# HyeonwooNoh/VQA-Transfer-ExternalData

Hardware: AMD Instinct MI355X
Metric: VQA train samples/sec (img+question) at bs512 (higher is better)
Workload: dtype f32

## Files before the change

include/vqa_hot.h:

```cpp
#ifndef VQA_HOT_H
#define VQA_HOT_H

#include <stdint.h>

#ifdef __cplusplus
extern "C" {
#endif

#define VQA_HOT_ABI_VERSION 5

enum {
    VQA_OK = 0,
    VQA_ERR_ARG = -1,
    VQA_ERR_ALIGN = -2,
    VQA_ERR_LAUNCH = -3,
    VQA_ERR_UNSUPPORTED = -4,
    VQA_ERR_WORKSPACE = -5
};

int vqa_hot_version(void);
const char* vqa_hot_error_string(int code);

int vqa_gather_features(const float* table, const int32_t* nbox_table, const int64_t* idx,
                        float* V, int32_t* nb, int B, int R, int D, int64_t N, void* stream);
// ... 8 lines not shown
int vqa_gru_unpack_dwx_bias(const float* dwx, float* gwg, float* gwc, float* gbg, float* gbc, int W, int H, void* stream);
int vqa_set_deterministic(int on);
int vqa_embed_bwd(const float* dx_tm, const int32_t* q, float* dE, int B, int T, int W, int Vq, void* stream);
int vqa_embed_bwd_len(const float* dx_tm, const int32_t* q, const int32_t* len, float* dE, int B, int T, int W,
                      int Vq, void* stream);
int vqa_embed_bwd_len_det(const float* dx_tm, const int32_t* q, const int32_t* len, float* dE, int B, int T, int W,
                          int Vq, int deterministic, void* stream);

int vqa_gemm_f32(int transA, int transB, int M, int N, int K, const float* A, int lda, const float* B,
                 int ldb, float* C, int ldc, const float* bias, const float* D, int ldd, int split_k,
                 float* workspace, int64_t workspace_floats, void* stream);
int vqa_gemm_f32_ex(int transA, int transB, int M, int N, int K, const float* A, int lda, const float* B,
                    int ldb, float* C, int ldc, const float* bias, const float* D, int ldd, int split_k,
                    float* workspace, int64_t workspace_floats, int max_blocks, void* stream);
int vqa_gemm_f32_gather(int M, int N, int K, const float* table, int lda, const int64_t* idx, int R,
                        int64_t n_samples_in_table, const float* B, int ldb, float* C, int ldc, const float* bias,
                        float* gathered_out, int ldg, void* stream);
int vqa_gemm_set_max_blocks(int n);
int vqa_gemm_set_order(int order);
int64_t vqa_gemm_workspace_floats(int transA, int transB, int M, int N, int K, int split_k);
int vqa_gemm_set_config(int cfg);
int vqa_gemm_set_gru_config(int cfg);
int vqa_gemm_set_tall_config(int cfg);

int vqa_ln_set_fast(int on);
int vqa_ln_relu_fwd(const float* pre, const float* gamma, const float* beta, const uint8_t* keepmask,
                    float keep_prob, float* y, float* mean, float* rstd, int G, int rows, int N, void* stream);
int vqa_ln_relu_bwd(const float* dy, const float* pre, const float* mean, const float* rstd,
                    const float* gamma, const float* beta, const uint8_t* keepmask, float keep_prob,
                    float* dpre, float* part_dgamma, float* part_dbeta, float* part_dbias, int G, int rows,
                    int N, void* stream);
int vqa_ln_act_fwd(const float* pre, const float* gamma, const float* beta, const uint8_t* keepmask, float keep_prob,
                   float* y, float* mean, float* rstd, int G, int rows, int N, int act, void* stream);
int vqa_ln_act_bwd(const float* dy, const float* pre, const float* mean, const float* rstd, const float* gamma,
                   const float* beta, const uint8_t* keepmask, float keep_prob, float* dpre, float* part_dgamma,
                   float* part_dbeta, float* part_dbias, int G, int rows, int N, int act, void* stream);
int vqa_ln_pair_mul_supported(int N, const void* const* ptrs, int n_ptrs);
int vqa_ln_pair_mul_fwd(const float* pre_a, const float* pre_b, const float* gamma_a, const float* beta_a, const float* gamma_b,
                        const float* beta_b, float* y_a, float* y_b, float* z, float* mean_a, float* rstd_a, float* mean_b,
                        float* rstd_b, int G, int N, void* stream);
int vqa_ln_pair_mul_bwd(const float* dz, const float* add_b, const float* pre_a, const float* pre_b, const float* mean_a,
                        const float* rstd_a, const float* mean_b, const float* rstd_b, const float* gamma_a, const float* beta_a,
                        const float* gamma_b, const float* beta_b, float* dpre_a, float* dpre_b, float* part_dgamma_a,
                        float* part_dbeta_a, float* part_dbias_a, float* part_dgamma_b, float* part_dbeta_b, float* part_dbias_b,
                        int G, int N, void* stream);
int vqa_tanh_fwd(const float* x, float* y, int64_t n, void* stream);
// ... 593 lines not shown
```

vqa-transfer-externaldata_amd/_lib.py:

```python
from __future__ import annotations

import ctypes as C
import os

_HERE = os.path.dirname(os.path.abspath(__file__))
_LIB_PATH = os.path.join(_HERE, "libvqahot.so")


class VqaHotError(RuntimeError):
    pass


def lib_path():
    return _LIB_PATH


class Dims(C.Structure):
    _fields_ = [("B", C.c_int32), ("R", C.c_int32), ("D", C.c_int32), ("H", C.c_int32), ("T", C.c_int32),
                ("W", C.c_int32), ("A", C.c_int32), ("Vq", C.c_int32), ("N_img", C.c_int64),
                ("model_type", C.c_int32), ("keep_att", C.c_float), ("keep_joint", C.c_float),
                ("inv_global_batch", C.c_float), ("flags", C.c_int32),
                ("num_marginal", C.c_int32), ("ent_cols", C.c_int32), ("extra_weight", C.c_float),
                ("map_dim", C.c_int32), ("La", C.c_int32)]

# ... 131 lines not shown


_P, _I, _L, _F, _U = C.c_void_p, C.c_int, C.c_int64, C.c_float, C.c_uint64

SIGNATURES = {
    "vqa_hot_version": (_I, []),
    "vqa_hot_error_string": (C.c_char_p, [_I]),
    "vqa_gather_features": (_I, [_P, _P, _P, _P, _P, _I, _I, _I, _L, _P]),
    "vqa_gather_features_bf16": (_I, [_P, _P, _P, _P, _P, _I, _I, _I, _L, _P]),
    "vqa_embed_fwd": (_I, [_P, _P, _P, _I, _I, _I, _I, _P]),
    "vqa_gru_pack_wx": (_I, [_P, _P, _P, _P, _P, _P, _I, _I, _P]),
    "vqa_gru_unpack_dwx": (_I, [_P, _P, _P, _I, _I, _P]),
    "vqa_embed_fwd_ld": (_I, [_P, _P, _P, _I, _I, _I, _I, _I, _P]),
    "vqa_gru_unpack_dwx_bias": (_I, [_P, _P, _P, _P, _P, _I, _I, _P]),
    "vqa_embed_bwd": (_I, [_P, _P, _P, _I, _I, _I, _I, _P]),
    "vqa_embed_bwd_len": (_I, [_P, _P, _P, _P, _I, _I, _I, _I, _P]),
    "vqa_embed_bwd_len_det": (_I, [_P, _P, _P, _P, _I, _I, _I, _I, _I, _P]),
    "vqa_set_deterministic": (_I, [_I]),
    "vqa_gemm_f32": (_I, [_I, _I, _I, _I, _I, _P, _I, _P, _I, _P, _I, _P, _P, _I, _I, _P, _L, _P]),
    "vqa_gemm_workspace_floats": (_L, [_I, _I, _I, _I, _I, _I]),
    "vqa_gemm_f32_ex": (_I, [_I, _I, _I, _I, _I, _P, _I, _P, _I, _P, _I, _P, _P, _I, _I, _P, _L, _I, _P]),
    "vqa_gemm_f32_gather": (_I, [_I, _I, _I, _P, _I, _P, _I, _L, _P, _I, _P, _I, _P, _P, _I, _P]),
    "vqa_gemm_set_tall_config": (_I, [_I]),
    "vqa_gemm_set_max_blocks": (_I, [_I]),
    "vqa_gemm_set_order": (_I, [_I]),
    "vqa_gemm_set_config": (_I, [_I]),
    "vqa_conv_set_config": (_I, [_I]),
    "vqa_gemm_set_gru_config": (_I, [_I]),
    "vqa_gru_seq_fwd": (_I, [_P, _P, _P, _P, _P, _P, _P, _P, _P, _I, _I, _I, _P]),
    "vqa_gru_seq_fwd_persistent": (_I, [_P, _P, _P, _P, _P, _P, _P, _P, _P, _I, _I, _I, _P, _P]),
    "vqa_gru_fwd_persistent_supported": (_I, [_I, _I, _I]),
    "vqa_gru_persistent_sync_bytes": (_L, []),
    "vqa_gru_set_persistent": (_I, [_I]),
    "vqa_gru_persistent_set_census": (_I, [_P]),
    "vqa_gru_seq_fwd_ws": (_I, [_P, _P, _P, _P, _P, _P, _P, _P, _P, _I, _I, _I, _P, _P]),
    "vqa_gru_seq_fwd_ws_ex": (_I, [_P, _P, _P, _P, _P, _P, _P, _P, _P, _I, _I, _I, _I, _P, _P]),
    "vqa_gru_ws_supported": (_I, [_I, _I, _I]),
    "vqa_gru_seq_bwd_ws": (_I, [_P, _P, _P, _P, _P, _P, _P, _P, _P, _P, _I, _I, _I, _P, _P]),
    "vqa_gru_seq_bwd_ws_ex": (_I, [_P, _P, _P, _P, _P, _P, _P, _P, _P, _P, _I, _I, _I, _I, _P, _P]),
    "vqa_gru_ws_bwd_supported": (_I, [_I, _I, _I]),
    "vqa_gru_ws_workspace_bytes": (_L, [_I]),
    "vqa_gru_ws_set_mode": (_I, [_I]),
    "vqa_gru_ws_set_form": (_I, [_I]),
    "vqa_gru_ws_set_stamps": (_I, [_P]),
    "vqa_gru_seq_fwd_rows": (_I, [_P, _P, _P, _P, _P, _P, _P, _P, _P, _I, _I, _I, _I, _I, _P]),
    "vqa_gru_seq_bwd_rows": (_I, [_P, _P, _P, _P, _P, _P, _P, _P, _P, _P, _I, _I, _I, _I, _I, _P]),
# ... 204 lines not shown
```

vqa-transfer-externaldata_amd/csrc/fusion_model.hip:

```cpp
#include <stdlib.h>
#include <string.h>

#include <string>
#include <vector>

#include "gru_encoder.h"
#include "keep_launch.h"

namespace {

inline bool has_tuned_head(int mt) { return mt == VQA_MODEL_VQA_ALL2 || mt == VQA_MODEL_VQA_ALL; }
inline bool train_loss_masked(int mt) { return mt != VQA_MODEL_STANDARD; }
inline bool bf16_routed(int mt) { return mt == VQA_MODEL_VLMAP_ANSWER || mt == VQA_MODEL_STANDARD; }
inline bool feat16(const vqa_dims_t& d) { return (d.flags & VQA_FLAG_BF16_FEATURES) != 0; }

void legacy_vqa_layout(Layout& L, const vqa_dims_t& d, int64_t& gw);

Layout make_layout(const vqa_dims_t& d) {
    Layout L;
    const int64_t B = d.B, R = d.R, D = d.D, H = d.H, T = d.T, W = d.W, A = d.A;
    L.add("V_ft", B * R * D, feat16(d) ? 2 : 4);
    L.add("num_V_ft", B);
    L.add("pre_v", B * R * H);
    L.add("v_linear_v", B * R * H);
    L.add("mean_v", B); L.add("rstd_v", B);
    const int64_t Wp = x_stride(W);
    L.add("x_tm", T * B * Wp);
    L.add("xp", T * B * 3 * H);
// ... 156 lines not shown
int g_h0skip_mode = -1;
inline int h0skip_mode() {
    if (g_h0skip_mode < 0) {
        const char* e = getenv("VQA_HOT_GRU_H0SKIP");
        g_h0skip_mode = e == nullptr ? 1 : (atoi(e) & 3);
    }
    return g_h0skip_mode;
}
int side_max_blocks() {
    static int v = -1;
    if (v < 0) {
        const char* e = getenv("VQA_HOT_SIDE_BLOCKS");
        v = e ? atoi(e) : 0;
    }
    return v;
}
int gather_mode(const vqa_dims_t* dims) {
    static int env = -2;
    if (env == -2) {
        const char* e = getenv("VQA_HOT_GATHER");
        env = e == nullptr ? -1 : (strcmp(e, "fused") == 0 ? 1 : 0);
    }
    if (env >= 0) return env;
    return (dims->flags & VQA_FLAG_FUSED_GATHER) ? 1 : 0;
}

struct Side {
    hipStream_t s = nullptr;
    hipEvent_t fork = nullptr, join = nullptr;
    bool ok = false, tried = false;
};
Side& side_stream() {
    static Side sd[64];
    int dev = 0;
    (void)hipGetDevice(&dev);
    Side& x = sd[dev & 63];
    if (!x.tried) {
        x.tried = true;
        const char* env = getenv("VQA_HOT_OVERLAP");
        if (env != nullptr && env[0] == '1') {
            x.ok = hipStreamCreateWithFlags(&x.s, hipStreamNonBlocking) == hipSuccess &&
                   hipEventCreateWithFlags(&x.fork, hipEventDisableTiming) == hipSuccess &&
                   hipEventCreateWithFlags(&x.join, hipEventDisableTiming) == hipSuccess;
        }
    }
    return x;
}
// ... 372 lines not shown

    Ctx side_ctx() const { return Ctx{{L, c.ws}, d, forked ? sd->s : c.st, forked ? 1 : 0}; }
    float* const dh = c.f("d_h0");
};

int side_record(const Step& s) { return !s.forked || join_side_record(*s.sd) ? VQA_OK : VQA_ERR_LAUNCH; }
int side_wait(const Step& s) {
    return !s.forked || hipStreamWaitEvent(s.c.st, s.sd->join, 0) == hipSuccess ? VQA_OK : VQA_ERR_LAUNCH;
}

enum GruForm { GRU_WS, GRU_LIVE, GRU_CHAINS };
enum GruDir { GRU_FWD, GRU_BWD };
GruForm gru_form(GruDir dir, int64_t T, int64_t B, int64_t H, const int32_t* live_rows) {
    const bool ws_ok = gru_ws_on() && (live_rows == nullptr || (T > 0 && live_rows[T - 1] > 0));
    if (ws_ok && (dir == GRU_FWD ? vqa_gru_ws_supported((int)T, (int)B, (int)H) : vqa_gru_ws_bwd_supported((int)T, (int)B, (int)H)) == 1)
        return GRU_WS;
    return live_rows != nullptr ? GRU_LIVE : GRU_CHAINS;
}


void fwd_visual_plan(Step& s) {
    s.sd = &side_stream();
    s.forked = fork_side(s.c, *s.sd);
    s.fuse_gather = !(s.d.flags & VQA_FLAG_BF16_GEMM) && gather_mode(&s.d) == 1 && (s.D % 32 == 0) && (s.H % 4 == 0) &&
                    vqa_aligned16(s.bt->table);
    s.visual_late = !s.forked && visual_late_enabled();
}

int fwd_visual(const Step& s) {
    const Ctx cv = s.side_ctx();
    const vqa_params_t* P = s.P;
    const vqa_batch_t* bt = s.bt;
    const int64_t B = s.B, R = s.R, D = s.D, H = s.H;
    {
        ProbeScope ps("gather", cv.st);
        if (feat16(s.d))
            TRY(vqa_gather_features_bf16(reinterpret_cast<const uint16_t*>(bt->table), bt->nbox_table, bt->image_idx,
                                         cv.u16("V_ft"), cv.i32("num_V_ft"), (int)B, (int)R, (int)D, s.d.N_img, cv.st));
        else
            TRY(vqa_gather_features(bt->table, bt->nbox_table, bt->image_idx, s.fuse_gather ? nullptr : cv.f("V_ft"),
                                    cv.i32("num_V_ft"), (int)B, (int)R, (int)D, s.d.N_img, cv.st));
    }
    if (s.fuse_gather) {
        {
            ProbeScope ps("v_linear_v.fwd_gemm", cv.st);
            TRY(vqa_gemm_f32_gather((int)(B * R), (int)H, (int)D, bt->table, (int)D, bt->image_idx, (int)R, s.d.N_img,
                                    P->v_linear_v.w, (int)H, cv.f("pre_v"), (int)H, P->v_linear_v.b, cv.f("V_ft"), (int)D,
// ... 609 lines not shown
```

vqa-transfer-externaldata_amd/csrc/gemm_args.h:

```cpp
#pragma once
#include <hip/hip_runtime.h>
#include <stdint.h>

struct GemmArgs {
    int M, N, K;
    const float* A; int lda;
    const float* B; int ldb;
    float* C; int ldc;
    const float* bias;
    const float* D; int ldd;
    int k_per_split;
    int64_t slab_stride;
    int vecA, vecB;
    int tiles_m, tiles_n, nsplit;
    int m_fastest;
    unsigned a_bytes, b_bytes;
    const float* scale;
    int relu;
    int Hi, Wi, Ci, Ho, Wo, cstride, pad_t, pad_l, kw;
    int conv_taps;
    int vec_epi;
    const int64_t* g_idx; int g_R; int64_t g_N; float* g_out; int g_ldo;
};

enum { EPI_PLAIN = 0, EPI_GATES = 1, EPI_CAND = 2, EPI_BWD_RH = 3, EPI_BWD_DH = 4 };
struct EpiArgs {
    int H, t, ldo;
    const int32_t* len;
    const float* h_prev;
    const float* i0;
    const float* i1;
    float* o0;
    float* o1;
    float* o2;
};

GemmArgs vqa_gemm_make_args(int M, int N, int K, const float* A, int lda, const float* B, int ldb, float* C, int ldc,
                            const float* bias, const float* D, int ldd);
int vqa_gru_step_launch(int epi, int cfg, const GemmArgs& a, const EpiArgs& ep, hipStream_t st);
int vqa_gru_rs_launch(int epi, const GemmArgs& a, const EpiArgs& ep, hipStream_t st);
```

vqa-transfer-externaldata_amd/csrc/gemm_f32.hip:

```cpp

#include "vqa_common.h"
#include "gemm_args.h"
#include <cstdio>
#include <cstdlib>

#ifndef VQA_GEMM_STAGGER
#define VQA_GEMM_STAGGER 1
#endif

typedef float f32x16 __attribute__((ext_vector_type(16)));
typedef unsigned int u32x4 __attribute__((ext_vector_type(4)));

#if defined(VQA_DBG_STAMPS)
__device__ unsigned long long* g_dbg_stamps = nullptr;
#define DBG_STAMP(i) do { if (threadIdx.x == 0) dbg_t[i] = __builtin_amdgcn_s_memrealtime(); } while (0)
#else
#define DBG_STAMP(i) do {} while (0)
#endif

namespace {


__device__ __forceinline__ int xcd_remap(int lin, int total) {
    const int q = total >> 3, r = total & 7;
// ... 153 lines not shown
                    const int k = idx / QPR, rq = (idx % QPR) * 4;
                    *reinterpret_cast<float4*>(s + k * BR + rq) = reg[i];
                }
            }
        }
    }
};

template <int BR, int BK, bool KC>
constexpr int tile_floats() { return KC ? BR * (BK + 4) : BK * BR; }

template <int BR, int BK, bool KC>
__device__ __forceinline__ float4 frag4(const float* s, int r0, int c, int lane) {
    const int i = lane & 31, h = lane >> 5;
    if (KC) {
        return *reinterpret_cast<const float4*>(s + (r0 + i) * (BK + 4) + c * 8 + h * 4);
    } else {
        const float* p = s + (c * 8 + h * 4) * BR + r0 + i;
        return make_float4(p[0], p[BR], p[2 * BR], p[3 * BR]);
    }
}

template <int BM, int BN, int WM, int WN, int WGK, int BK, int DEEP, bool A_KC, bool B_KC, int EPI, bool CONV = false,
          bool EDGE = false, int NT = 256, bool GATHER = false>
__global__ __launch_bounds__(NT, (CONV && NT == 256) ? 4 : 1) void gemm_f32_kernel(GemmArgs p, EpiArgs ep) {
    static_assert(!GATHER || (A_KC && DEEP == 0 && !CONV && !EDGE && EPI == EPI_PLAIN), "row-gathered A: plain NN/NT tiles");
    constexpr int TM = WM / 32, TN = WN / 32;
    constexpr int WAVES_M = BM / WM, WAVES_N = BN / WN;
    static_assert(WAVES_M * WAVES_N * WGK * 64 == NT, "one 32x32-tiled wave per (m, n, k-group) slot");
    static_assert((BK / 8) % WGK == 0, "k chunks split evenly over the k wave groups");
    constexpr int A_FL = tile_floats<BM, BK, A_KC>();
    constexpr int B_FL = tile_floats<BN, BK, B_KC>();
    extern __shared__ __attribute__((aligned(16))) float smem[];

    if (EPI != EPI_PLAIN) __builtin_amdgcn_s_setprio(3);
#if defined(VQA_DBG_STAMPS)
    unsigned long long dbg_t[8] = {0, 0, 0, 0, 0, 0, 0, 0};
    if (threadIdx.x == 0) dbg_t[5] = __builtin_amdgcn_s_memtime();
#endif
    DBG_STAMP(0);
    const int lane = threadIdx.x & 63, wave = threadIdx.x >> 6;
    const int wk = wave / (WAVES_M * WAVES_N);
    const int wm = (wave / WAVES_N) % WAVES_M, wn = wave % WAVES_N;
    const int tiles_mn = p.tiles_m * p.tiles_n;
    const int total = tiles_mn * p.nsplit;
    for (int lin = blockIdx.x; lin < total; lin += gridDim.x) {
    const int tile = xcd_remap(lin, total);
    const int bz = tile / tiles_mn, bmn = tile - bz * tiles_mn;
    const int m0 = (p.m_fastest ? bmn % p.tiles_m : bmn / p.tiles_n) * BM;
// ... 93 lines not shown
        Stager<BN, BK, B_KC, NT> sb;
        constexpr int NVA = Stager<BM, BK, A_KC, NT>::NV;
        int iy0[NVA], ix0[NVA], pix[NVA];
        if (CONV) {
#pragma unroll
            for (int i = 0; i < NVA; ++i) {
                const int idx = threadIdx.x + i * NT;
                const int m = m0 + idx / (BK / 4);
                pix[i] = -1; iy0[i] = ix0[i] = 0;
                if (idx < BM * (BK / 4) && m < p.M) {
                    const int hw = p.Ho * p.Wo;
                    const int b = m / hw, r = m - b * hw;
                    const int oy = r / p.Wo, ox = r - oy * p.Wo;
                    iy0[i] = oy * p.cstride - p.pad_t;
                    ix0[i] = ox * p.cstride - p.pad_l;
                    pix[i] = b * p.Hi * p.Wi;
                }
            }
        }
        const float* gsrc[NVA];
        unsigned gdst[NVA];
        const bool g_store = GATHER && p.g_out != nullptr && n0 == 0;
        const __amdgpu_buffer_rsrc_t rsG = __builtin_amdgcn_make_buffer_rsrc(
            p.g_out, 0, GATHER && p.g_out != nullptr ? (int)(((int64_t)(p.M - 1) * p.g_ldo + p.K) * 4) : 0, 0x00020000);
        if (GATHER) {
#pragma unroll
            for (int i = 0; i < NVA; ++i) {
                const int idx = threadIdx.x + i * NT;
                const int row = idx / (BK / 4), kq = (idx % (BK / 4)) * 4;
                const int m = m0 + row, mc = min(m, p.M - 1);
                const int smp = mc / p.g_R, reg_row = mc - smp * p.g_R;
                int64_t src = p.g_idx[smp];
                src = src < 0 ? 0 : (src >= p.g_N ? p.g_N - 1 : src);
                gsrc[i] = p.A + (src * p.g_R + reg_row) * (int64_t)p.lda + kq;
                gdst[i] = (m < p.M) ? (unsigned)(((int64_t)m * p.g_ldo + kq) * 4) : Stager<BM, BK, A_KC, NT>::OOB;
            }
        }
        auto load_a = [&](int k0) {
            if (GATHER) sa.load_ptr(gsrc, k0 - kbeg);
            else if (CONV) sa.load_conv(rsA, iy0, ix0, pix, k0, p.Hi, p.Wi, p.Ci, p.kw);
            else if (EDGE) sa.load(p.A, p.lda, m0, k0, p.M, kend, va);
            else sa.load_fast(rsA, p.lda, m0, k0, p.M, kend);
        };
        auto load_b = [&](int k0) {
            if (EDGE) sb.load(p.B, p.ldb, n0, k0, p.N, kend, vb);
            else sb.load_fast(rsB, p.ldb, n0, k0, p.N, kend);
        };
        if (nt > 0) {
            load_a(kbeg);
            load_b(kbeg);
            sa.store(L0);
            sb.store(L0 + A_FL);
            if (g_store) sa.store_buf(rsG, gdst, 0u);
        }
        __syncthreads();
        int t = 0;
        if (CONV && p.conv_taps <= 32 && p.Ci % BK == 0) {
            unsigned cbase[NVA], cmask[NVA];
            const int kh = p.conv_taps / p.kw;
#pragma unroll
            for (int i = 0; i < NVA; ++i) {
                const int idx = threadIdx.x + i * NT;
// ... 18 lines not shown
            };
            if (c0 >= p.Ci) { c0 = 0; tap = 1; if (++kx == p.kw) { kx = 0; ++ky; } }
            for (; t + 2 < nt; t += 2) {
                sa.load_conv_full(rsA, cbase, cmask, (unsigned)(((ky * p.Wi + kx) * p.Ci + c0) * 4), 1u << tap);
                sb.load_full(rsB, ob);
                ob += stepB; advance();
                __builtin_amdgcn_sched_barrier(0);
                compute_tile(L0, L0 + A_FL);
                __builtin_amdgcn_sched_barrier(0);
                sa.store(L1);
                sb.store(L1 + A_FL);
                __syncthreads();
                sa.load_conv_full(rsA, cbase, cmask, (unsigned)(((ky * p.Wi + kx) * p.Ci + c0) * 4), 1u << tap);
                sb.load_full(rsB, ob);
                ob += stepB; advance();
                __builtin_amdgcn_sched_barrier(0);
                compute_tile(L1, L1 + A_FL);
                __builtin_amdgcn_sched_barrier(0);
                sa.store(L0);
                sb.store(L0 + A_FL);
                __syncthreads();
            }
        }
        if (!CONV && !EDGE) {
            sa.init_full(p.lda, m0, kbeg, p.M);
            sb.init_full(p.ldb, n0, kbeg, p.N);
            const unsigned stepA = (unsigned)(A_KC ? BK : BK * p.lda) * 4u;
            const unsigned stepB = (unsigned)(B_KC ? BK : BK * p.ldb) * 4u;
            const int nfull = (kend - kbeg) / BK;
            unsigned oa = stepA, ob = stepB;
            constexpr bool STAG = (NT == 512) && !GATHER && EPI == EPI_PLAIN && (VQA_GEMM_STAGGER != 0) &&
                                  ((WM == 32 && WN == 32 && BK == 32 && BM + BN == 192) || (BM == 128 && BN == 128 && BK == 16));
            const bool stag_wg = STAG && nfull >= 16;
            if (stag_wg && wave >= 4) {
                sa.load_full(rsA, oa); sb.load_full(rsB, ob);
                oa += stepA; ob += stepB;
                for (; t + 3 < nfull; t += 2) {
                    sa.store(L1); sb.store(L1 + A_FL);
                    sa.load_full(rsA, oa); sb.load_full(rsB, ob);
                    oa += stepA; ob += stepB;
                    __builtin_amdgcn_sched_barrier(0);
                    compute_tile(L0, L0 + A_FL);
                    __builtin_amdgcn_sched_barrier(0);
                    __syncthreads();
                    sa.store(L0); sb.store(L0 + A_FL);
                    sa.load_full(rsA, oa); sb.load_full(rsB, ob);
                    oa += stepA; ob += stepB;
                    __builtin_amdgcn_sched_barrier(0);
                    compute_tile(L1, L1 + A_FL);
                    __builtin_amdgcn_sched_barrier(0);
                    __syncthreads();
                }
                sa.store(L1); sb.store(L1 + A_FL);
                __builtin_amdgcn_sched_barrier(0);
                compute_tile(L0, L0 + A_FL);
                __builtin_amdgcn_sched_barrier(0);
                __syncthreads();
                ++t;
            } else if (stag_wg) {
                for (; t + 3 < nfull; t += 2) {
                    sa.load_full(rsA, oa); sb.load_full(rsB, ob);
                    oa += stepA; ob += stepB;
                    __builtin_amdgcn_sched_barrier(0);
                    compute_tile(L0, L0 + A_FL);
                    __builtin_amdgcn_sched_barrier(0);
                    sa.store(L1); sb.store(L1 + A_FL);
                    __syncthreads();
                    sa.load_full(rsA, oa); sb.load_full(rsB, ob);
                    oa += stepA; ob += stepB;
                    __builtin_amdgcn_sched_barrier(0);
                    compute_tile(L1, L1 + A_FL);
                    __builtin_amdgcn_sched_barrier(0);
                    sa.store(L0); sb.store(L0 + A_FL);
                    __syncthreads();
                }
                sa.load_full(rsA, oa); sb.load_full(rsB, ob);
                __builtin_amdgcn_sched_barrier(0);
                compute_tile(L0, L0 + A_FL);
                __builtin_amdgcn_sched_barrier(0);
                sa.store(L1); sb.store(L1 + A_FL);
                __syncthreads();
                ++t;
            }
            for (; !stag_wg && t + 2 < nfull; t += 2) {
                if (GATHER) sa.load_ptr(gsrc, (t + 1) * BK); else sa.load_full(rsA, oa);
                sb.load_full(rsB, ob);
                oa += stepA; ob += stepB;
                __builtin_amdgcn_sched_barrier(0);
                compute_tile(L0, L0 + A_FL);
                __builtin_amdgcn_sched_barrier(0);
                sa.store(L1);
                sb.store(L1 + A_FL);
                if (g_store) sa.store_buf(rsG, gdst, (unsigned)((t + 1) * BK) * 4u);
                __syncthreads();
                if (GATHER) sa.load_ptr(gsrc, (t + 2) * BK); else sa.load_full(rsA, oa);
                sb.load_full(rsB, ob);
                oa += stepA; ob += stepB;
                __builtin_amdgcn_sched_barrier(0);
                compute_tile(L1, L1 + A_FL);
                __builtin_amdgcn_sched_barrier(0);
                sa.store(L0);
                sb.store(L0 + A_FL);
                if (g_store) sa.store_buf(rsG, gdst, (unsigned)((t + 2) * BK) * 4u);
                __syncthreads();
            }
        }
        for (; t + 1 < nt; ++t) {
            float* cur = (t & 1) ? L1 : L0;
            float* nxt = (t & 1) ? L0 : L1;
            load_a(kbeg + (t + 1) * BK);
            load_b(kbeg + (t + 1) * BK);
            __builtin_amdgcn_sched_barrier(0);
            compute_tile(cur, cur + A_FL);
            __builtin_amdgcn_sched_barrier(0);
            sa.store(nxt);
            sb.store(nxt + A_FL);
            if (g_store) sa.store_buf(rsG, gdst, (unsigned)((t + 1) * BK) * 4u);
            __syncthreads();
        }
        if (nt > 0) {
            float* cur = ((nt - 1) & 1) ? L1 : L0;
            compute_tile(cur, cur + A_FL);
            __syncthreads();
        }
    } else {
        Stager<BM, BK, A_KC, NT> sa0, sa1;
        Stager<BN, BK, B_KC, NT> sb0, sb1;
        auto ld0 = [&](int tile) {
            sa0.load_fast(rsA, p.lda, m0, kbeg + tile * BK, p.M, kend);
            sb0.load_fast(rsB, p.ldb, n0, kbeg + tile * BK, p.N, kend);
        };
        auto ld1 = [&](int tile) {
            sa1.load_fast(rsA, p.lda, m0, kbeg + tile * BK, p.M, kend);
            sb1.load_fast(rsB, p.ldb, n0, kbeg + tile * BK, p.N, kend);
        };
        auto st0 = [&]() { sa0.store(L0); sb0.store(L0 + A_FL); };
        auto st1 = [&]() { sa1.store(L1); sb1.store(L1 + A_FL); };
        if (nt > 0) ld0(0);
        if (nt > 1) ld1(1);
        if (nt > 0) st0();
        __syncthreads();
        DBG_STAMP(1);
        int t = 0;
        {
            sa0.init_full(p.lda, m0, kbeg, p.M); sa1.init_full(p.lda, m0, kbeg, p.M);
            sb0.init_full(p.ldb, n0, kbeg, p.N); sb1.init_full(p.ldb, n0, kbeg, p.N);
// ... 273 lines not shown
        unsigned long long* o = g_dbg_stamps + ((size_t)EPI * 4096 + blockIdx.x) * 8;
        for (int i = 0; i < 7; ++i) o[i] = dbg_t[i];
    }
#endif
}

__global__ __launch_bounds__(256) void splitk_reduce_kernel(const float* __restrict__ slabs, float* __restrict__ C,
                                                            int M, int N, int ldc, int S) {
    const int64_t n4 = (int64_t)M * N / 4;
    for (int64_t i = blockIdx.x * 256 + threadIdx.x; i < n4; i += (int64_t)gridDim.x * 256) {
        float4 a = reinterpret_cast<const float4*>(slabs)[i];
        for (int z = 1; z < S; ++z) {
            const float4 b = reinterpret_cast<const float4*>(slabs + (int64_t)z * M * N)[i];
            a.x += b.x; a.y += b.y; a.z += b.z; a.w += b.w;
        }
        const int64_t e = i * 4;
        const int row = (int)(e / N), col = (int)(e % N);
        float* c = C + (int64_t)row * ldc + col;
        c[0] = a.x; c[1] = a.y; c[2] = a.z; c[3] = a.w;
    }
}

template <int BM, int BN, int WM, int WN, int WGK, int BK, int DEEP, bool A_KC, bool B_KC, int EPI, bool CONV = false,
          bool EDGE = false, int NT = 256, bool GATHER = false>
int launch_one(GemmArgs a, const EpiArgs& ep, int split, hipStream_t st, int max_blocks = 0) {
    constexpr size_t tiles = 2 * (tile_floats<BM, BK, A_KC>() + tile_floats<BN, BK, B_KC>()) * sizeof(float);
    constexpr size_t red = (EPI == EPI_PLAIN) ? (size_t)(WGK - 1) * (BM / WM) * (BN / WN) * (WM / 32) * (WN / 32) * 16 * 64 * sizeof(float) : 0;
    constexpr size_t stage = (size_t)(EPI == EPI_PLAIN ? 1 : WGK) * (BM / WM) * (BN / WN) * 32 * 36 * sizeof(float);
    constexpr size_t lds = tiles > red + stage ? tiles : red + stage;
    auto kern = gemm_f32_kernel<BM, BN, WM, WN, WGK, BK, DEEP, A_KC, B_KC, EPI, CONV, EDGE, NT, GATHER>;
    static bool attr_done = false;
    if (lds > 64 * 1024 && !attr_done) {
        if (hipFuncSetAttribute(reinterpret_cast<const void*>(kern), hipFuncAttributeMaxDynamicSharedMemorySize,
                                (int)lds) != hipSuccess)
            return VQA_ERR_LAUNCH;
        attr_done = true;
    }
    a.tiles_m = (a.M + BM - 1) / BM;
    a.tiles_n = (a.N + BN - 1) / BN;
    a.nsplit = split;
    {
        const double per_xcd = (double)a.tiles_m * a.tiles_n / 8.0;
        auto foot = [&](double t_fast, double t_slow, double b_fast, double b_slow) {
            const double slow_panels = std::min(t_slow, per_xcd / t_fast + 1.0);
            const double fast_panels = std::min(t_fast, per_xcd);
            return slow_panels * b_slow + fast_panels * b_fast;
        };
// ... 94 lines not shown
        case 4: return launch_one<64, 64, 32, 32, 1, 64, false, true, BKC, EPI>(a, ep, 1, st);
        case 7: return launch_one<64, 32, 32, 32, 2, 64, false, true, BKC, EPI>(a, ep, 1, st);
        case 8: return launch_one<32, 32, 32, 32, 4, 64, false, true, BKC, EPI>(a, ep, 1, st);
        case 9: return launch_one<32, 64, 32, 32, 2, 64, false, true, BKC, EPI>(a, ep, 1, st);
        case 10: return launch_one<64, 64, 32, 32, 1, 64, true, true, BKC, EPI>(a, ep, 1, st);
        case 11: return launch_one<64, 32, 32, 32, 2, 64, true, true, BKC, EPI>(a, ep, 1, st);
        case 12: return launch_one<64, 64, 32, 32, 1, 32, true, true, BKC, EPI>(a, ep, 1, st);
        case 13: return launch_one<64, 32, 32, 32, 2, 32, true, true, BKC, EPI>(a, ep, 1, st);
        case 16: return launch_one<32, 32, 32, 32, 4, 32, true, true, BKC, EPI>(a, ep, 1, st);
        case 20: return launch_one<128, 64, 32, 32, 1, 32, 0, true, BKC, EPI, false, false, 512>(a, ep, 1, st);
        case 21: return launch_one<64, 128, 32, 32, 1, 32, 0, true, BKC, EPI, false, false, 512>(a, ep, 1, st);
        case 17: return launch_one<64, 32, 32, 32, 4, 32, 1, true, BKC, EPI, false, false, 512>(a, ep, 1, st);
        case 18:
            if (EPI == EPI_GATES) return launch_one<64, 64, 32, 32, 4, 64, 1, true, BKC, EPI, false, false, 1024>(a, ep, 1, st);
            return launch_one<64, 32, 32, 32, 8, 64, 1, true, BKC, EPI, false, false, 1024>(a, ep, 1, st);
        default: return VQA_ERR_ARG;
    }
}

inline int64_t cdiv(int64_t a, int64_t b) { return (a + b - 1) / b; }

int g_force_cfg = -1;
int g_tall_cfg = 20;
int g_max_blocks = 0;
int g_conv_cfg = -1;
int g_conv_cfg_plain = -1;

inline int tall_small_cfg() {
    static const int v = vqa_env_int("VQA_HOT_TALL_SMALL_CFG", 12);
    return v < NUM_CFG ? v : 12;
}

inline int tune_pair(const char* env, int cfg, int split) {
    const char* e = getenv(env);
    if (e != nullptr) {
        int c = 0, s = 0;
        if (sscanf(e, "%d:%d", &c, &s) == 2 && c >= 0 && c < NUM_CFG && s >= 0 && s <= 16) { cfg = c; split = s; }
    }
    return (cfg << 8) | split;
}

void choose(int tA, int tB, int M, int N, int K, int& cfg, int& split) {
    int64_t target;
    if (tA) {
        static const int tn_short = vqa_env_int("VQA_HOT_TN_SHORT_CFG", 20);
        static const int tn_mid = vqa_env_int("VQA_HOT_TN_MID_CFG", 20);
// ... 160 lines not shown
        const int grid = (int)std::min<int64_t>(cdiv(n4, 256), 2048);
        hipLaunchKernelGGL(splitk_reduce_kernel, dim3(grid), dim3(256), 0, st, workspace, C, M, N, ldc, split);
        VQA_CHECK_LAUNCH();
        return VQA_OK;
    }
    a.k_per_split = (int)cdiv(std::max(K, 1), 64) * 64;
    return launch_by_id(cfg, transA, transB, a, 1, st, max_blocks);
}

extern "C" int vqa_gemm_f32_gather(int M, int N, int K, const float* table, int lda, const int64_t* idx, int R,
                                   int64_t n_samples_in_table, const float* B, int ldb, float* C, int ldc,
                                   const float* bias, float* gathered_out, int ldg, void* stream) {
    VQA_REQUIRE(M >= 0 && N >= 0 && K > 0 && R > 0 && n_samples_in_table > 0, VQA_ERR_ARG);
    if (M == 0 || N == 0) return VQA_OK;
    VQA_REQUIRE(table && idx && B && C, VQA_ERR_ARG);
    VQA_REQUIRE(lda >= K && ldb >= N && ldc >= N && (gathered_out == nullptr || ldg >= K), VQA_ERR_ARG);
    VQA_REQUIRE(K % 32 == 0 && N % 4 == 0, VQA_ERR_UNSUPPORTED);
    VQA_REQUIRE(lda % 4 == 0 && vqa_aligned16(table) && ldb % 4 == 0 && vqa_aligned16(B) &&
                    (gathered_out == nullptr || (ldg % 4 == 0 && vqa_aligned16(gathered_out))),
                VQA_ERR_ALIGN);
    GemmArgs a = vqa_gemm_make_args(M, N, K, table, lda, B, ldb, C, ldc, bias, nullptr, 0);
    const int64_t bb = ((int64_t)(K - 1) * ldb + N) * 4;
    VQA_REQUIRE(bb < 0xFFFFFF00ll, VQA_ERR_UNSUPPORTED);
    a.a_bytes = 0;
    a.b_bytes = (unsigned)bb;
    VQA_REQUIRE(gathered_out == nullptr || ((int64_t)(M - 1) * ldg + K) * 4 < 0xFFFFFF00ll, VQA_ERR_UNSUPPORTED);
    a.g_idx = idx; a.g_R = R; a.g_N = n_samples_in_table; a.g_out = gathered_out; a.g_ldo = ldg;
    a.k_per_split = (int)cdiv(K, 64) * 64;
    const EpiArgs ep{};
    hipStream_t st = static_cast<hipStream_t>(stream);
    if (g_tall_cfg == 21)
        return launch_one<64, 128, 32, 32, 1, 32, 0, true, false, EPI_PLAIN, false, false, 512, true>(a, ep, 1, st, 0);
    return launch_one<128, 64, 32, 32, 1, 32, 0, true, false, EPI_PLAIN, false, false, 512, true>(a, ep, 1, st, 0);
}

extern "C" int vqa_gemm_set_tall_config(int cfg) {
    VQA_REQUIRE(cfg == 20 || cfg == 21, VQA_ERR_ARG);
    g_tall_cfg = cfg;
    return VQA_OK;
}

extern "C" int vqa_conv2d_nhwc(const float* x, int B, int Hi, int Wi, int Ci, const float* w, int kh, int kw, int Co,
                               int stride, int pad_t, int pad_l, int Ho, int Wo, const float* scale,
                               const float* shift, const float* residual, int relu, float* y, void* stream) {
    VQA_REQUIRE(x && w && y && B > 0 && Hi > 0 && Wi > 0 && Ci > 0 && Co > 0 && kh > 0 && kw > 0 && stride > 0 &&
                    Ho > 0 && Wo > 0,
                VQA_ERR_ARG);
    VQA_REQUIRE((int64_t)B * Ho * Wo < (1ll << 31) && (int64_t)B * Hi * Wi < (1ll << 31), VQA_ERR_ARG);
    hipStream_t st = static_cast<hipStream_t>(stream);
    const int M = B * Ho * Wo, K = kh * kw * Ci;
    const bool plain = (kh == 1 && kw == 1 && stride == 1 && pad_t == 0 && pad_l == 0 && Ho == Hi && Wo == Wi);
    GemmArgs a = vqa_gemm_make_args(M, Co, K, x, Ci, w, Co, y, Co, shift, residual, Co);
    a.scale = scale;
    a.relu = relu;
    if (plain && (shortk_mode() & 2) && Ci >= 128 && Ci <= 256 && Co >= 2 * Ci && g_conv_cfg_plain < 0 && g_force_cfg < 0 &&
        vqa_gemm_shortk_supported(M, Co, K, Ci, Co, Co) && vqa_aligned16(x) && vqa_aligned16(w) &&
// ... 35 lines not shown
```

Baseline: 164,000.

## Fuse row gather into GEMM via buffer offsets and enable by default

Adds a gather GEMM variant that loads gathered A rows through buffer-resource offsets, so the table rows share the same staggered, pipelined k-loop as the plain GEMM instead of going through per-thread pointer loads. The k-loop is moved into an include file so it can be specialised for the offset gather, pointer gather and plain paths. The default gather mode now fuses the gather into the GEMM whenever the plain heuristic would pick the same tall config, which removes the separate gather kernel and the extra pass over memory for the features. The risk is that gathered rows are scattered, so A loads coalesce less well, and the table must fit within the 32-bit buffer offset range.

```diff
diff --git a/include/vqa_hot.h b/include/vqa_hot.h
--- a/include/vqa_hot.h
+++ b/include/vqa_hot.h
@@ -54,6 +54,7 @@
 int vqa_gemm_set_config(int cfg);
 int vqa_gemm_set_gru_config(int cfg);
 int vqa_gemm_set_tall_config(int cfg);
+int vqa_gemm_set_gather_ptr(int on);
 
 int vqa_ln_set_fast(int on);
 int vqa_ln_relu_fwd(const float* pre, const float* gamma, const float* beta, const uint8_t* keepmask,
diff --git a/vqa-transfer-externaldata_amd/_lib.py b/vqa-transfer-externaldata_amd/_lib.py
--- a/vqa-transfer-externaldata_amd/_lib.py
+++ b/vqa-transfer-externaldata_amd/_lib.py
@@ -177,6 +177,7 @@
     "vqa_gemm_f32_ex": (_I, [_I, _I, _I, _I, _I, _P, _I, _P, _I, _P, _I, _P, _P, _I, _I, _P, _L, _I, _P]),
     "vqa_gemm_f32_gather": (_I, [_I, _I, _I, _P, _I, _P, _I, _L, _P, _I, _P, _I, _P, _P, _I, _P]),
     "vqa_gemm_set_tall_config": (_I, [_I]),
+    "vqa_gemm_set_gather_ptr": (_I, [_I]),
     "vqa_gemm_set_max_blocks": (_I, [_I]),
     "vqa_gemm_set_order": (_I, [_I]),
     "vqa_gemm_set_config": (_I, [_I]),
diff --git a/vqa-transfer-externaldata_amd/csrc/fusion_model.hip b/vqa-transfer-externaldata_amd/csrc/fusion_model.hip
--- a/vqa-transfer-externaldata_amd/csrc/fusion_model.hip
+++ b/vqa-transfer-externaldata_amd/csrc/fusion_model.hip
@@ -4,6 +4,7 @@
 #include <string>
 #include <vector>
 
+#include "gemm_args.h"
 #include "gru_encoder.h"
 #include "keep_launch.h"
 
@@ -206,7 +207,7 @@
         env = e == nullptr ? -1 : (strcmp(e, "fused") == 0 ? 1 : 0);
     }
     if (env >= 0) return env;
-    return (dims->flags & VQA_FLAG_FUSED_GATHER) ? 1 : 0;
+    return (dims->flags & VQA_FLAG_FUSED_GATHER) ? 1 : 2;
 }
 
 struct Side {
@@ -625,7 +626,10 @@
 void fwd_visual_plan(Step& s) {
     s.sd = &side_stream();
     s.forked = fork_side(s.c, *s.sd);
-    s.fuse_gather = !(s.d.flags & VQA_FLAG_BF16_GEMM) && gather_mode(&s.d) == 1 && (s.D % 32 == 0) && (s.H % 4 == 0) &&
+    const int gm = gather_mode(&s.d);
+    const bool same_kernel = gm == 2 && side_max_blocks() == 0 &&
+                             vqa_gemm_gather_matches_plain((int)(s.B * s.R), (int)s.H, (int)s.D, (int)s.D, (int)s.R, s.d.N_img);
+    s.fuse_gather = !(s.d.flags & VQA_FLAG_BF16_GEMM) && (gm == 1 || same_kernel) && (s.D % 32 == 0) && (s.H % 4 == 0) &&
                     vqa_aligned16(s.bt->table);
     s.visual_late = !s.forked && visual_late_enabled();
 }
diff --git a/vqa-transfer-externaldata_amd/csrc/gemm_args.h b/vqa-transfer-externaldata_amd/csrc/gemm_args.h
--- a/vqa-transfer-externaldata_amd/csrc/gemm_args.h
+++ b/vqa-transfer-externaldata_amd/csrc/gemm_args.h
@@ -37,5 +37,6 @@
 
 GemmArgs vqa_gemm_make_args(int M, int N, int K, const float* A, int lda, const float* B, int ldb, float* C, int ldc,
                             const float* bias, const float* D, int ldd);
+bool vqa_gemm_gather_matches_plain(int M, int N, int K, int lda, int R, int64_t n_samples_in_table);
 int vqa_gru_step_launch(int epi, int cfg, const GemmArgs& a, const EpiArgs& ep, hipStream_t st);
 int vqa_gru_rs_launch(int epi, const GemmArgs& a, const EpiArgs& ep, hipStream_t st);
diff --git a/vqa-transfer-externaldata_amd/csrc/gemm_f32.hip b/vqa-transfer-externaldata_amd/csrc/gemm_f32.hip
--- a/vqa-transfer-externaldata_amd/csrc/gemm_f32.hip
+++ b/vqa-transfer-externaldata_amd/csrc/gemm_f32.hip
@@ -199,9 +199,10 @@
 }
 
 template <int BM, int BN, int WM, int WN, int WGK, int BK, int DEEP, bool A_KC, bool B_KC, int EPI, bool CONV = false,
-          bool EDGE = false, int NT = 256, bool GATHER = false>
+          bool EDGE = false, int NT = 256, int GATHER = 0>
 __global__ __launch_bounds__(NT, (CONV && NT == 256) ? 4 : 1) void gemm_f32_kernel(GemmArgs p, EpiArgs ep) {
     static_assert(!GATHER || (A_KC && DEEP == 0 && !CONV && !EDGE && EPI == EPI_PLAIN), "row-gathered A: plain NN/NT tiles");
+    static_assert(!GATHER || Stager<BM, BK, A_KC, NT>::EXACT, "row-gathered A: every thread owns whole float4s of the tile");
     constexpr int TM = WM / 32, TN = WN / 32;
     constexpr int WAVES_M = BM / WM, WAVES_N = BN / WN;
     static_assert(WAVES_M * WAVES_N * WGK * 64 == NT, "one 32x32-tiled wave per (m, n, k-group) slot");
@@ -341,7 +342,7 @@
         unsigned gdst[NVA];
         const bool g_store = GATHER && p.g_out != nullptr && n0 == 0;
         const __amdgpu_buffer_rsrc_t rsG = __builtin_amdgcn_make_buffer_rsrc(
-            p.g_out, 0, GATHER && p.g_out != nullptr ? (int)(((int64_t)(p.M - 1) * p.g_ldo + p.K) * 4) : 0, 0x00020000);
+            p.g_out, 0, g_store ? (int)(((int64_t)(p.M - 1) * p.g_ldo + p.K) * 4) : 0, 0x00020000);
         if (GATHER) {
 #pragma unroll
             for (int i = 0; i < NVA; ++i) {
@@ -351,12 +352,15 @@
                 const int smp = mc / p.g_R, reg_row = mc - smp * p.g_R;
                 int64_t src = p.g_idx[smp];
                 src = src < 0 ? 0 : (src >= p.g_N ? p.g_N - 1 : src);
-                gsrc[i] = p.A + (src * p.g_R + reg_row) * (int64_t)p.lda + kq;
+                const int64_t el = (src * p.g_R + reg_row) * (int64_t)p.lda + kq;
+                gsrc[i] = p.A + el;
+                if (GATHER == 2) sa.voff[i] = (unsigned)(el * 4);
                 gdst[i] = (m < p.M) ? (unsigned)(((int64_t)m * p.g_ldo + kq) * 4) : Stager<BM, BK, A_KC, NT>::OOB;
             }
         }
         auto load_a = [&](int k0) {
-            if (GATHER) sa.load_ptr(gsrc, k0 - kbeg);
+            if (GATHER == 2) sa.load_full(rsA, (unsigned)(k0 - kbeg) * 4u);
+            else if (GATHER) sa.load_ptr(gsrc, k0 - kbeg);
             else if (CONV) sa.load_conv(rsA, iy0, ix0, pix, k0, p.Hi, p.Wi, p.Ci, p.kw);
             else if (EDGE) sa.load(p.A, p.lda, m0, k0, p.M, kend, va);
             else sa.load_fast(rsA, p.lda, m0, k0, p.M, kend);
@@ -421,106 +425,14 @@
                 __syncthreads();
             }
         }
-        if (!CONV && !EDGE) {
-            sa.init_full(p.lda, m0, kbeg, p.M);
-            sb.init_full(p.ldb, n0, kbeg, p.N);
-            const unsigned stepA = (unsigned)(A_KC ? BK : BK * p.lda) * 4u;
-            const unsigned stepB = (unsigned)(B_KC ? BK : BK * p.ldb) * 4u;
-            const int nfull = (kend - kbeg) / BK;
-            unsigned oa = stepA, ob = stepB;
-            constexpr bool STAG = (NT == 512) && !GATHER && EPI == EPI_PLAIN && (VQA_GEMM_STAGGER != 0) &&
-                                  ((WM == 32 && WN == 32 && BK == 32 && BM + BN == 192) || (BM == 128 && BN == 128 && BK == 16));
-            const bool stag_wg = STAG && nfull >= 16;
-            if (stag_wg && wave >= 4) {
-                sa.load_full(rsA, oa); sb.load_full(rsB, ob);
-                oa += stepA; ob += stepB;
-                for (; t + 3 < nfull; t += 2) {
-                    sa.store(L1); sb.store(L1 + A_FL);
-                    sa.load_full(rsA, oa); sb.load_full(rsB, ob);
-                    oa += stepA; ob += stepB;
-                    __builtin_amdgcn_sched_barrier(0);
-                    compute_tile(L0, L0 + A_FL);
-                    __builtin_amdgcn_sched_barrier(0);
-                    __syncthreads();
-                    sa.store(L0); sb.store(L0 + A_FL);
-                    sa.load_full(rsA, oa); sb.load_full(rsB, ob);
-                    oa += stepA; ob += stepB;
-                    __builtin_amdgcn_sched_barrier(0);
-                    compute_tile(L1, L1 + A_FL);
-                    __builtin_amdgcn_sched_barrier(0);
-                    __syncthreads();
-                }
-                sa.store(L1); sb.store(L1 + A_FL);
-                __builtin_amdgcn_sched_barrier(0);
-                compute_tile(L0, L0 + A_FL);
-                __builtin_amdgcn_sched_barrier(0);
-                __syncthreads();
-                ++t;
-            } else if (stag_wg) {
-                for (; t + 3 < nfull; t += 2) {
-                    sa.load_full(rsA, oa); sb.load_full(rsB, ob);
-                    oa += stepA; ob += stepB;
-                    __builtin_amdgcn_sched_barrier(0);
-                    compute_tile(L0, L0 + A_FL);
-                    __builtin_amdgcn_sched_barrier(0);
-                    sa.store(L1); sb.store(L1 + A_FL);
-                    __syncthreads();
-                    sa.load_full(rsA, oa); sb.load_full(rsB, ob);
-                    oa += stepA; ob += stepB;
-                    __builtin_amdgcn_sched_barrier(0);
-                    compute_tile(L1, L1 + A_FL);
-                    __builtin_amdgcn_sched_barrier(0);
-                    sa.store(L0); sb.store(L0 + A_FL);
-                    __syncthreads();
-                }
-                sa.load_full(rsA, oa); sb.load_full(rsB, ob);
-                __builtin_amdgcn_sched_barrier(0);
-                compute_tile(L0, L0 + A_FL);
-                __builtin_amdgcn_sched_barrier(0);
-                sa.store(L1); sb.store(L1 + A_FL);
-                __syncthreads();
-                ++t;
-            }
-            for (; !stag_wg && t + 2 < nfull; t += 2) {
-                if (GATHER) sa.load_ptr(gsrc, (t + 1) * BK); else sa.load_full(rsA, oa);
-                sb.load_full(rsB, ob);
-                oa += stepA; ob += stepB;
-                __builtin_amdgcn_sched_barrier(0);
-                compute_tile(L0, L0 + A_FL);
-                __builtin_amdgcn_sched_barrier(0);
-                sa.store(L1);
-                sb.store(L1 + A_FL);
-                if (g_store) sa.store_buf(rsG, gdst, (unsigned)((t + 1) * BK) * 4u);
-                __syncthreads();
-                if (GATHER) sa.load_ptr(gsrc, (t + 2) * BK); else sa.load_full(rsA, oa);
-                sb.load_full(rsB, ob);
-                oa += stepA; ob += stepB;
-                __builtin_amdgcn_sched_barrier(0);
-                compute_tile(L1, L1 + A_FL);
-                __builtin_amdgcn_sched_barrier(0);
-                sa.store(L0);
-                sb.store(L0 + A_FL);
-                if (g_store) sa.store_buf(rsG, gdst, (unsigned)((t + 2) * BK) * 4u);
-                __syncthreads();
-            }
-        }
-        for (; t + 1 < nt; ++t) {
-            float* cur = (t & 1) ? L1 : L0;
-            float* nxt = (t & 1) ? L0 : L1;
-            load_a(kbeg + (t + 1) * BK);
-            load_b(kbeg + (t + 1) * BK);
-            __builtin_amdgcn_sched_barrier(0);
-            compute_tile(cur, cur + A_FL);
-            __builtin_amdgcn_sched_barrier(0);
-            sa.store(nxt);
-            sb.store(nxt + A_FL);
-            if (g_store) sa.store_buf(rsG, gdst, (unsigned)((t + 1) * BK) * 4u);
-            __syncthreads();
-        }
-        if (nt > 0) {
-            float* cur = ((nt - 1) & 1) ? L1 : L0;
-            compute_tile(cur, cur + A_FL);
-            __syncthreads();
+        if (GATHER == 2 && g_store) {
+#define VQA_KLOOPS_GS true
+#include "gemm_f32_kloops.inc"
+#undef VQA_KLOOPS_GS
+        } else {
+#define VQA_KLOOPS_GS (GATHER == 1 && g_store)
+#include "gemm_f32_kloops.inc"
+#undef VQA_KLOOPS_GS
         }
     } else {
         Stager<BM, BK, A_KC, NT> sa0, sa1;
@@ -840,7 +752,7 @@
 }
 
 template <int BM, int BN, int WM, int WN, int WGK, int BK, int DEEP, bool A_KC, bool B_KC, int EPI, bool CONV = false,
-          bool EDGE = false, int NT = 256, bool GATHER = false>
+          bool EDGE = false, int NT = 256, int GATHER = 0>
 int launch_one(GemmArgs a, const EpiArgs& ep, int split, hipStream_t st, int max_blocks = 0) {
     constexpr size_t tiles = 2 * (tile_floats<BM, BK, A_KC>() + tile_floats<BN, BK, B_KC>()) * sizeof(float);
     constexpr size_t red = (EPI == EPI_PLAIN) ? (size_t)(WGK - 1) * (BM / WM) * (BN / WN) * (WM / 32) * (WN / 32) * 16 * 64 * sizeof(float) : 0;
@@ -981,6 +893,7 @@
 
 int g_force_cfg = -1;
 int g_tall_cfg = 20;
+bool g_gather_ptr = false;
 int g_max_blocks = 0;
 int g_conv_cfg = -1;
 int g_conv_cfg_plain = -1;
@@ -1187,7 +1100,9 @@
     GemmArgs a = vqa_gemm_make_args(M, N, K, table, lda, B, ldb, C, ldc, bias, nullptr, 0);
     const int64_t bb = ((int64_t)(K - 1) * ldb + N) * 4;
     VQA_REQUIRE(bb < 0xFFFFFF00ll, VQA_ERR_UNSUPPORTED);
-    a.a_bytes = 0;
+    const int64_t ab = ((n_samples_in_table * R - 1) * (int64_t)lda + K) * 4;
+    const bool by_offset = !g_gather_ptr && ab < 0xFFFFFF00ll;
+    a.a_bytes = by_offset ? (unsigned)ab : 0;
     a.b_bytes = (unsigned)bb;
     VQA_REQUIRE(gathered_out == nullptr || ((int64_t)(M - 1) * ldg + K) * 4 < 0xFFFFFF00ll, VQA_ERR_UNSUPPORTED);
     a.g_idx = idx; a.g_R = R; a.g_N = n_samples_in_table; a.g_out = gathered_out; a.g_ldo = ldg;
@@ -1195,8 +1110,23 @@
     const EpiArgs ep{};
     hipStream_t st = static_cast<hipStream_t>(stream);
     if (g_tall_cfg == 21)
-        return launch_one<64, 128, 32, 32, 1, 32, 0, true, false, EPI_PLAIN, false, false, 512, true>(a, ep, 1, st, 0);
-    return launch_one<128, 64, 32, 32, 1, 32, 0, true, false, EPI_PLAIN, false, false, 512, true>(a, ep, 1, st, 0);
+        return by_offset ? launch_one<64, 128, 32, 32, 1, 32, 0, true, false, EPI_PLAIN, false, false, 512, 2>(a, ep, 1, st, 0)
+                         : launch_one<64, 128, 32, 32, 1, 32, 0, true, false, EPI_PLAIN, false, false, 512, 1>(a, ep, 1, st, 0);
+    return by_offset ? launch_one<128, 64, 32, 32, 1, 32, 0, true, false, EPI_PLAIN, false, false, 512, 2>(a, ep, 1, st, 0)
+                     : launch_one<128, 64, 32, 32, 1, 32, 0, true, false, EPI_PLAIN, false, false, 512, 1>(a, ep, 1, st, 0);
+}
+
+extern "C" int vqa_gemm_set_gather_ptr(int on) {
+    g_gather_ptr = on != 0;
+    return VQA_OK;
+}
+
+bool vqa_gemm_gather_matches_plain(int M, int N, int K, int lda, int R, int64_t n_samples_in_table) {
+    if (bf16x3_mode() || g_gather_ptr || K % 32 != 0 || N % 4 != 0) return false;
+    if (((n_samples_in_table * R - 1) * (int64_t)lda + K) * 4 >= 0xFFFFFF00ll) return false;
+    int cfg, split = 0;
+    choose(0, 0, M, N, K, cfg, split);
+    return cfg == g_tall_cfg && split == 1 && M >= 2048 && N >= 512 && K >= 2048;
 }
 
 extern "C" int vqa_gemm_set_tall_config(int cfg) {
diff --git a/vqa-transfer-externaldata_amd/csrc/gemm_f32_kloops.inc b/vqa-transfer-externaldata_amd/csrc/gemm_f32_kloops.inc
--- /dev/null
+++ b/vqa-transfer-externaldata_amd/csrc/gemm_f32_kloops.inc
@@ -0,0 +1,100 @@
+        if (!CONV && !EDGE) {
+            if (!GATHER) sa.init_full(p.lda, m0, kbeg, p.M);
+            sb.init_full(p.ldb, n0, kbeg, p.N);
+            const unsigned stepA = (unsigned)(A_KC ? BK : BK * p.lda) * 4u;
+            const unsigned stepB = (unsigned)(B_KC ? BK : BK * p.ldb) * 4u;
+            const int nfull = (kend - kbeg) / BK;
+            unsigned oa = stepA, ob = stepB;
+            auto fetch_ab = [&](int tile) {
+                if (GATHER == 1) sa.load_ptr(gsrc, tile * BK); else sa.load_full(rsA, oa);
+                sb.load_full(rsB, ob);
+                oa += stepA; ob += stepB;
+            };
+            auto put_g = [&]() { if (VQA_KLOOPS_GS) sa.store_buf(rsG, gdst, oa - stepA); };
+            constexpr bool STAG = (NT == 512) && GATHER != 1 && EPI == EPI_PLAIN && (VQA_GEMM_STAGGER != 0) &&
+                                  ((WM == 32 && WN == 32 && BK == 32 && BM + BN == 192) || (BM == 128 && BN == 128 && BK == 16));
+            const bool stag_wg = STAG && nfull >= 16;
+            if (stag_wg && wave >= 4) {
+                fetch_ab(1);
+                for (; t + 3 < nfull; t += 2) {
+                    sa.store(L1); sb.store(L1 + A_FL); put_g();
+                    fetch_ab(t + 2);
+                    __builtin_amdgcn_sched_barrier(0);
+                    compute_tile(L0, L0 + A_FL);
+                    __builtin_amdgcn_sched_barrier(0);
+                    __syncthreads();
+                    sa.store(L0); sb.store(L0 + A_FL); put_g();
+                    fetch_ab(t + 3);
+                    __builtin_amdgcn_sched_barrier(0);
+                    compute_tile(L1, L1 + A_FL);
+                    __builtin_amdgcn_sched_barrier(0);
+                    __syncthreads();
+                }
+                sa.store(L1); sb.store(L1 + A_FL); put_g();
+                __builtin_amdgcn_sched_barrier(0);
+                compute_tile(L0, L0 + A_FL);
+                __builtin_amdgcn_sched_barrier(0);
+                __syncthreads();
+                ++t;
+            } else if (stag_wg) {
+                for (; t + 3 < nfull; t += 2) {
+                    fetch_ab(t + 1);
+                    __builtin_amdgcn_sched_barrier(0);
+                    compute_tile(L0, L0 + A_FL);
+                    __builtin_amdgcn_sched_barrier(0);
+                    sa.store(L1); sb.store(L1 + A_FL); put_g();
+                    __syncthreads();
+                    fetch_ab(t + 2);
+                    __builtin_amdgcn_sched_barrier(0);
+                    compute_tile(L1, L1 + A_FL);
+                    __builtin_amdgcn_sched_barrier(0);
+                    sa.store(L0); sb.store(L0 + A_FL); put_g();
+                    __syncthreads();
+                }
+                if (GATHER == 1) sa.load_ptr(gsrc, (t + 1) * BK); else sa.load_full(rsA, oa);
+                sb.load_full(rsB, ob);
+                __builtin_amdgcn_sched_barrier(0);
+                compute_tile(L0, L0 + A_FL);
+                __builtin_amdgcn_sched_barrier(0);
+                sa.store(L1); sb.store(L1 + A_FL);
+                if (VQA_KLOOPS_GS) sa.store_buf(rsG, gdst, oa);
+                __syncthreads();
+                ++t;
+            }
+            for (; !stag_wg && t + 2 < nfull; t += 2) {
+                fetch_ab(t + 1);
+                __builtin_amdgcn_sched_barrier(0);
+                compute_tile(L0, L0 + A_FL);
+                __builtin_amdgcn_sched_barrier(0);
+                sa.store(L1);
+                sb.store(L1 + A_FL);
+                put_g();
+                __syncthreads();
+                fetch_ab(t + 2);
+                __builtin_amdgcn_sched_barrier(0);
+                compute_tile(L1, L1 + A_FL);
+                __builtin_amdgcn_sched_barrier(0);
+                sa.store(L0);
+                sb.store(L0 + A_FL);
+                put_g();
+                __syncthreads();
+            }
+        }
+        for (; t + 1 < nt; ++t) {
+            float* cur = (t & 1) ? L1 : L0;
+            float* nxt = (t & 1) ? L0 : L1;
+            load_a(kbeg + (t + 1) * BK);
+            load_b(kbeg + (t + 1) * BK);
+            __builtin_amdgcn_sched_barrier(0);
+            compute_tile(cur, cur + A_FL);
+            __builtin_amdgcn_sched_barrier(0);
+            sa.store(nxt);
+            sb.store(nxt + A_FL);
+            if (VQA_KLOOPS_GS) sa.store_buf(rsG, gdst, (unsigned)((t + 1) * BK) * 4u);
+            __syncthreads();
+        }
+        if (nt > 0) {
+            float* cur = ((nt - 1) & 1) ? L1 : L0;
+            compute_tile(cur, cur + A_FL);
+            __syncthreads();
+        }
```

After: 166,000 (median of 6 runs). 1.2% higher.
